# jaehyuck0103/OpenMAVIS

Hardware: AMD Instinct MI355X
Metric: multi-cam frames/sec (ORB extract+match) + LocalBA iters/sec, 5x720x540 (higher is better)
Workload: dtype u8

## Files before the change

include/omv.h:

```cpp
#ifndef OMV_H
#define OMV_H

#include <stddef.h>
#include <stdint.h>

#ifdef __cplusplus
extern "C" {
#endif

typedef int omv_status;
#define OMV_OK 0
#define OMV_ERR_ARG 1
#define OMV_ERR_HIP 2
#define OMV_ERR_CAPACITY 3
#define OMV_ERR_NO_DEVICE 4

typedef struct omv_orb_params {
    int nfeatures;
    float scale_factor;
    int nlevels;
    int ini_th_fast;
    int min_th_fast;
} omv_orb_params;

// ... 34 lines not shown
omv_status omv_orb_debug_level(omv_orb *orb, int img, int level, uint8_t *out, int *w, int *h);

typedef struct omv_frame_geom {
    int n_cams;
    float min_x, max_x;
    float min_y, max_y;
    int nlevels;
    float scale_factors[16];
    int cam_model[8];
} omv_frame_geom;

typedef struct omv_mp_view {
    const uint8_t *desc;
    const float *proj_x;
    const float *proj_y;
    const float *view_cos;
    const int32_t *level;
    const uint8_t *in_view;
    const float *track_depth;
    const uint8_t *is_bad;
    const uint8_t *has_obs;
} omv_mp_view;

typedef struct omv_matcher omv_matcher;

omv_status omv_matcher_create(int max_frames, int n_cams, int kp_cap, int max_mps, omv_matcher **out);
omv_status omv_matcher_destroy(omv_matcher *m);

omv_status omv_matcher_assign_grid(omv_matcher *m, int n_frames, const omv_frame_geom *geom, const omv_kp *kps,
                                   const int *n_kp, void *stream);
omv_status omv_matcher_grid_debug(omv_matcher *m, int frame, int cam, int32_t *cell_start, int32_t *idx);

omv_status omv_matcher_search_projection(omv_matcher *m, int n_frames, const omv_frame_geom *geom, const omv_kp *kps,
                                         const uint8_t *desc, const int *n_kp, const omv_mp_view *mps, int M, float th,
                                         int far_points, float th_far, float nnratio, const int32_t *l2r,
                                         const int32_t *r2l, const uint8_t *kp_occ_init, int32_t *kp_to_mp,
                                         int *n_matches, void *stream);

omv_status omv_matcher_stereo_lapping(omv_matcher *m, int n_frames, const uint8_t *desc, const int *n_kp,
                                      const int *mono, double ratio, int32_t *l2r, int32_t *r2l, void *stream);

omv_status omv_matcher_stereo_triangulate(omv_matcher *m, int n_frames, int n_cams, int kp_cap, const omv_kp *kps,
                                          const int *n_kp, const int *mono, const float *cams, const float *Rlr,
                                          const float *tlr, const float *level_sigma2, int nlevels, int32_t *l2r,
                                          int32_t *r2l, float *depth, float *p3d, void *stream);

omv_status omv_matcher_last_error(omv_matcher *m);

omv_status omv_matcher_enable_timing(omv_matcher *m, int on);
omv_status omv_matcher_stage_ms(omv_matcher *m, double *ms4, int reset);

omv_status omv_bf_knn2(int n_pairs, const uint8_t *query, int q_cap, const int *nq, const uint8_t *train, int t_cap,
                       const int *nt, int32_t *idx2, int32_t *dist2, void *stream);

typedef struct omv_se3f {
    float q[4];
    float t[3];
} omv_se3f;

typedef struct omv_last_frame {
    const float *pos;
    const uint8_t *desc;
    const uint8_t *valid;
    const uint8_t *has_obs;
    const omv_kp *kps;
    int S;
} omv_last_frame;

omv_status omv_matcher_search_last_frame(omv_matcher *m, int n_frames, const omv_frame_geom *geom, const omv_kp *kps,
                                         const uint8_t *desc, const int *n_kp, const float *cams, const omv_se3f *Tcw,
                                         const omv_se3f *Tlw, const omv_se3f *Trl, const omv_last_frame *last, float th,
                                         int bMono, float mb, int check_ori, const uint8_t *kp_occ_init,
                                         int32_t *kp_to_mp, int32_t *n_matches, void *stream);

enum { OMV_KF_FUSE = 0, OMV_KF_FUSE_SIM3 = 1, OMV_KF_SBP_SIM3 = 2, OMV_KF_SBP_FRAME = 3 };

typedef struct omv_kf_search_job {
    int kf;
    int cam;
    omv_se3f Tcw;
    float Ow[3];
    int mp_start, mp_count;
} omv_kf_search_job;

typedef struct omv_kf_mps {
    const float *pos;
    const float *normal;
    const float *min_dist;
    const float *max_dist;
    const uint8_t *desc;
} omv_kf_mps;

typedef struct omv_kf_search_params {
    int mode;
    float th;
    float max_dist;
    float bf;
    const float *uright;
    float inv_level_sigma2[16];
    float log_scale_factor;
    int n_levels;
    float cams[8][8];
    int check_ori;
    const float *mp_angle;
} omv_kf_search_params;

// ... 458 lines not shown
```

openmavis_amd/_lib.py:

```python
import ctypes
import os

_HERE = os.path.dirname(os.path.abspath(__file__))
LIB_PATH = os.path.join(_HERE, "libomv_hip.so")

OMV_OK = 0
OMV_ERR_ARG = 1
OMV_ERR_HIP = 2
OMV_ERR_CAPACITY = 3
OMV_ERR_NO_DEVICE = 4
CAM_KB8 = 0
CAM_PINHOLE = 1
_ERRS = {1: "bad argument", 2: "HIP runtime error", 3: "device capacity exceeded", 4: "no HIP device"}


class OmvError(RuntimeError):
    pass


def check(status, what="omv call"):
    if status != OMV_OK:
        raise OmvError(f"{what} failed: {_ERRS.get(status, status)} ({status})")


# ... 167 lines not shown

class FisheyeUndist(ctypes.Structure):
    _fields_ = [("K", ctypes.c_float * 4), ("D", ctypes.c_double * 4), ("newK", ctypes.c_float * 4)]


class LbaOpts(ctypes.Structure):
    _fields_ = [("opt_it", ctypes.c_int), ("lambda_init", ctypes.c_double), ("max_trials", ctypes.c_int),
                ("large", ctypes.c_int)]


class LbaResult(ctypes.Structure):
    _fields_ = [("err", ctypes.c_float), ("err_end", ctypes.c_float), ("status", ctypes.c_int),
                ("iterations", ctypes.c_int), ("trials", ctypes.c_int), ("lambda_", ctypes.c_double),
                ("mono_chi2", ctypes.c_void_p), ("mono_outlier", ctypes.c_void_p),
                ("stereo_chi2", ctypes.c_void_p), ("stereo_outlier", ctypes.c_void_p)]


try:
    import numpy as _np

    KP_DTYPE = _np.dtype([("x", "<f4"), ("y", "<f4"), ("size", "<f4"), ("angle", "<f4"),
                          ("response", "<f4"), ("octave", "<i4")])
except ImportError:
    KP_DTYPE = None

_VP, _I, _F, _SZ = ctypes.c_void_p, ctypes.c_int, ctypes.c_float, ctypes.c_size_t
ALLREDUCE_FN = ctypes.CFUNCTYPE(ctypes.c_int, ctypes.c_void_p, ctypes.c_void_p, ctypes.c_size_t, ctypes.c_void_p)
SIGNATURES = {
    "omv_orb_create": (_I, [ctypes.POINTER(OrbParams), _I, _I, _I, ctypes.POINTER(_VP)]),
    "omv_orb_destroy": (_I, [_VP]),
    "omv_selftest_node_sort": (_I, [_VP, _VP, _I, _VP, _VP]),
    "omv_orb_max_keypoints": (_I, [_VP]),
    "omv_orb_scale_tables": (_I, [_VP, _VP, _VP, _VP, _VP]),
    "omv_orb_extract_batch": (_I, [_VP, _I, _VP, _SZ, _SZ, _VP, _VP, _VP, _VP, _VP, _VP]),
    "omv_orb_extract_host": (_I, [_VP, _VP, _SZ, _I, _I, _VP, _VP, _VP, _VP]),
    "omv_orb_last_error": (_I, [_VP]),
    "omv_orb_enable_timing": (_I, [_VP, _I]),
    "omv_orb_set_harris": (_I, [_VP, _VP]),
    "omv_orb_stage_ms": (_I, [_VP, _VP, ctypes.POINTER(ctypes.c_longlong), _I]),
    "omv_orb_last_counts": (_I, [_VP, ctypes.POINTER(ctypes.c_longlong), ctypes.POINTER(ctypes.c_longlong)]),
    "omv_orb_debug_level": (_I, [_VP, _I, _I, _VP, ctypes.POINTER(_I), ctypes.POINTER(_I)]),
    "omv_matcher_create": (_I, [_I, _I, _I, _I, ctypes.POINTER(_VP)]),
    "omv_matcher_destroy": (_I, [_VP]),
    "omv_matcher_assign_grid": (_I, [_VP, _I, ctypes.POINTER(FrameGeom), _VP, _VP, _VP]),
    "omv_matcher_grid_debug": (_I, [_VP, _I, _I, _VP, _VP]),
    "omv_matcher_enable_timing": (_I, [_VP, _I]),
    "omv_matcher_last_error": (_I, [_VP]),
    "omv_matcher_stage_ms": (_I, [_VP, _VP, _I]),
    "omv_matcher_search_projection": (_I, [_VP, _I, ctypes.POINTER(FrameGeom), _VP, _VP, _VP,
                                           ctypes.POINTER(MpView), _I, _F, _I, _F, _F, _VP, _VP, _VP, _VP,
                                           _VP, _VP]),
    "omv_matcher_stereo_lapping": (_I, [_VP, _I, _VP, _VP, _VP, ctypes.c_double, _VP, _VP, _VP]),
    "omv_bf_knn2": (_I, [_I, _VP, _I, _VP, _VP, _I, _VP, _VP, _VP, _VP]),
    "omv_matcher_search_last_frame": (_I, [_VP, _I, ctypes.POINTER(FrameGeom), _VP, _VP, _VP, _VP, _VP, _VP,
                                           ctypes.POINTER(SE3f), ctypes.POINTER(LastFrame), _F, _I, _F, _I, _VP, _VP,
                                           _VP, _VP]),
    "omv_frustum": (_I, [_I, _VP, ctypes.POINTER(Rig), ctypes.POINTER(MpWorld), _I, _F, ctypes.POINTER(MpTrack), _VP,
                         _VP]),
    "omv_lba_create": (_I, [_I, _I, _I, _I, _I, ctypes.POINTER(_VP)]),
    "omv_lba_destroy": (_I, [_VP]),
    "omv_lba_set_problem": (_I, [_VP, ctypes.POINTER(LbaProblem)]),
    "omv_lba_optimize": (_I, [_VP, ctypes.POINTER(LbaOpts), ctypes.POINTER(LbaProblem), ctypes.POINTER(LbaResult)]),
    "omv_lba_evaluate": (_I, [_VP, _VP, _VP, _VP, _VP]),
    "omv_lba_evaluate_stereo": (_I, [_VP, _VP, _VP, _VP]),
    "omv_lba_stage_ms": (_I, [_VP, _VP, ctypes.POINTER(_I)]),
    "omv_lba_host_syncs": (_I, [_VP, ctypes.POINTER(_I), ctypes.POINTER(_I)]),
    "omv_lba_enable_timing": (_I, [_VP, _I]),
    "omv_lba_set_driver": (_I, [_VP, _I]),
    "omv_lba_reset": (_I, [_VP]),
    "omv_lba_set_comm": (_I, [_VP, _I, _I, _VP, _VP]),
    "omv_tri_debug": (_I, [_VP, _VP, _VP, _VP, _VP, _VP, _F, _F, _VP]),
    "omv_matcher_stereo_triangulate": (_I, [_VP, _I, _I, _I, _VP, _VP, _VP, _VP, _VP, _VP, _VP, _I, _VP, _VP, _VP,
                                            _VP, _VP]),
    "omv_matcher_search_for_triangulation": (_I, [_VP, _I, ctypes.POINTER(TriPair), _VP, _VP, _I, _I, _I, _VP, _VP]),
    "omv_matcher_search_by_bow": (_I, [_VP, _I, ctypes.POINTER(BowJob), _I, _F, _I, _VP, _VP]),
    "omv_matcher_bow_rescans": (_I, [ctypes.POINTER(ctypes.c_int64), _I]),
    "omv_matcher_search_for_initialization": (_I, [_VP, _I, _VP, ctypes.POINTER(FrameGeom), _VP, _VP, _VP, _VP, _I,
                                                   _F, _I, _VP, _VP, _VP]),
    "omv_pose_create": (_I, [_I, _I, ctypes.POINTER(_VP)]),
    "omv_pose_destroy": (_I, [_VP]),
    "omv_pose_inertial_last_kf": (_I, [_VP, ctypes.POINTER(PoseBatch), _I, _VP, _VP, _VP, _VP]),
    "omv_pose_inertial_last_frame": (_I, [_VP, ctypes.POINTER(PoseBatch), ctypes.POINTER(PosePrior), _I, _VP, _VP,
                                          _VP, _VP]),
    "omv_pose_constraint": (_I, [_I, _VP, _VP, _VP]),
    "omv_pose_optimization": (_I, [_VP, ctypes.POINTER(PoseBatch), _VP, _VP, _VP, _VP, _VP, _VP, _VP]),
    "omv_pose_set_mode": (_I, [_VP, _I, _I]),
    "omv_pose_edges_from_matches": (_I, [_VP, _I, _I, _VP, _VP, _VP, _VP, _VP, _VP, _I, _VP, _I] + [_VP] * 14),
    "omv_pose_last_error": (_I, [_VP, ctypes.POINTER(ctypes.c_int32), _VP]),
    "omv_matcher_search_kf": (_I, [_VP, _I, ctypes.POINTER(FrameGeom), _VP, _VP, _VP, _I, ctypes.POINTER(KfSearchJob),
                                   _I, _VP, ctypes.POINTER(KfMps), ctypes.POINTER(KfSearchParams), _VP, _VP, _VP, _VP,
                                   _VP]),
    "omv_search_in_neighbors_fuse": (_I, [_VP, ctypes.POINTER(FrameGeom), _VP, _VP, _VP, _I, ctypes.POINTER(FuseGraph),
                                          _I, _I, _VP, ctypes.POINTER(KfMps), ctypes.POINTER(KfSearchParams), _VP, _VP]),
    "omv_matcher_search_by_sim3": (_I, [_VP, _I, ctypes.POINTER(FrameGeom), _VP, _VP, _VP, _I, ctypes.POINTER(Sim3Job),
                                        _I, _VP, _VP, _I, _VP, _VP, ctypes.POINTER(KfMps), _F, _F, _I, _VP, _VP, _VP]),
    "omv_imu_preintegrate": (_I, [_I, _VP, _VP, _VP, _VP, _VP, _VP, _VP]),
    "omv_bow_transform": (_I, [ctypes.POINTER(Vocab), _I, _VP, _I, _VP, _I] + [_VP] * 10 + [_VP]),
    "omv_lba_shard": (_I, [_VP, ctypes.POINTER(ctypes.c_int32), ctypes.POINTER(ctypes.c_int32), _VP]),
    "omv_frame_uright": (_I, [_I, _I, _I, _I, _VP, _VP, _VP, _I, _I, ctypes.POINTER(FisheyeUndist), _F, _VP, _VP,
                              _VP]),
    "omv_frame_pack": (_I, [_I, _I, _I, _I, _VP, _VP, _VP, _VP, _VP, _VP, _VP, _VP, _VP]),
    "omv_mappoint_distinctive_descriptors": (_I, [_I, _VP, _VP, _VP, _VP, _VP, _VP]),
    "omv_create_new_map_points": (_I, [_I, _VP, _VP, _VP, _VP, _I, _I, _I, ctypes.c_float, ctypes.c_float, _I, _VP,
                                       _VP, _VP]),
    "omv_local_mapping_create_new_map_points": (_I, [_VP, _VP, _VP, _I, _VP, _VP, _VP, _I, _I, _I, _I, _I,
                                                     ctypes.c_float, ctypes.c_float, _VP, _VP, _VP]),
# ... 74 lines not shown
```

openmavis_amd/csrc/match.hip:

```cpp
#include <hip/hip_runtime.h>

#include <climits>
#include <cstdlib>
#include <cstring>
#include <type_traits>
#include <cmath>
#include <cstdio>
#include <vector>

#include "../../include/omv.h"
#include "omv_camera.h"
#include "omv_device.h"
#include "omv_host.h"

namespace {

constexpr int kGridCols = 64, kGridRows = 48, kCells = kGridCols * kGridRows;
constexpr int kTH_HIGH = 100;
constexpr int kTop = 16;
constexpr int kMaxCams = 8;
constexpr size_t kResolveLds = 150 * 1024;

struct FrameArgs {
    int n_cams, kp_cap, nlevels;
// ... 1070 lines not shown
    const int *q_off, *t_off;
    int pair_stride_off;
    int32_t *idx2, *dist2;
    int out_cap;
};

template <int G>
__global__ void __launch_bounds__(256) knn2_kernel(KnnArgs a, int n_pairs) {
    __shared__ __attribute__((aligned(16))) uint64_t tile[256][4];
    constexpr int QB = 256 / G;
    const int pair = blockIdx.y;
    const int qo = a.q_off ? a.q_off[pair * a.pair_stride_off] : 0;
    const int to = a.t_off ? a.t_off[pair * a.pair_stride_off] : 0;
    const int nq = a.nq[pair * a.pair_stride_off] - qo;
    const int nt = a.nt[pair * a.pair_stride_off] - to;
    const int g = threadIdx.x % G;
    const int qi = blockIdx.x * QB + threadIdx.x / G;
    if (blockIdx.x * QB >= max(nq, 0)) return;
    uint64_t dq[4] = {0, 0, 0, 0};
    if (qi < nq) omv::load_desc(a.q + pair * a.q_stride + (size_t)(qo + qi) * 32, dq);
    uint64_t k0 = ~0ull >> 1, k1 = ~0ull >> 1;
    int d0 = INT_MAX, d1 = INT_MAX, i0 = -1, i1 = -1;
    for (int b = 0; b < nt; b += 256) {
        __syncthreads();
        const int j = b + threadIdx.x;
        if (j < nt) omv::load_desc(a.t + pair * a.t_stride + (size_t)(to + j) * 32, tile[threadIdx.x]);
        __syncthreads();
        const int e = min(256, nt - b);
        for (int k = g; k < e; k += G) {
            const int d = omv::hamming256(dq, tile[k]);
            if (d < d1) {
                if (d0 > d) d1 = d0, i1 = i0, d0 = d, i0 = b + k;
                else d1 = d, i1 = b + k;
            }
        }
    }
    k0 = ((uint64_t)(uint32_t)d0 << 32) | (uint32_t)i0;
    k1 = ((uint64_t)(uint32_t)d1 << 32) | (uint32_t)i1;
#pragma unroll
    for (int m = 1; m < G; m <<= 1) {
        const uint64_t o0 = __shfl_xor(k0, m, 64), o1 = __shfl_xor(k1, m, 64);
        const uint64_t r0 = k0 < o0 ? k0 : o0;
        const uint64_t r1 = k0 < o0 ? (k1 < o0 ? k1 : o0) : (k0 < o1 ? k0 : o1);
        k0 = r0, k1 = r1;
    }
    if (qi < nq && g == 0) {
        int32_t *oi = a.idx2 + ((size_t)pair * a.out_cap + qi) * 2;
        int32_t *od = a.dist2 + ((size_t)pair * a.out_cap + qi) * 2;
        oi[0] = (int32_t)(uint32_t)k0, oi[1] = (int32_t)(uint32_t)k1;
        od[0] = (int32_t)(k0 >> 32), od[1] = (int32_t)(k1 >> 32);
    }
}

static void launch_knn2(const KnnArgs &a, int n_pairs, int q_cap, hipStream_t st) {
    if ((long long)n_pairs * q_cap <= 4096)
        knn2_kernel<32><<<dim3((q_cap + 7) / 8, n_pairs), 256, 0, st>>>(a, n_pairs);
    else
        knn2_kernel<8><<<dim3((q_cap + 31) / 32, n_pairs), 256, 0, st>>>(a, n_pairs);
}

__global__ void stereo_pairs_kernel(const int32_t *idx2, const int32_t *dist2, int out_cap, const int *n_kp,
                                    const int *mono, int n_cams, int kp_cap, double ratio, int32_t *l2r,
                                    int32_t *r2l, int n_frames) {
    const int frame = blockIdx.y;
    const int q = blockIdx.x * blockDim.x + threadIdx.x;
    if (q >= kp_cap) return;
    const int m0 = mono[frame * n_cams], m1 = mono[frame * n_cams + 1];
    const int nq = n_kp[frame * n_cams] - m0, qi = q - m0;
    int32_t v = -1;
    if (qi >= 0 && qi < nq) {
        const int32_t *oi = idx2 + ((size_t)frame * out_cap + qi) * 2;
        const int32_t *od = dist2 + ((size_t)frame * out_cap + qi) * 2;
        if (oi[1] >= 0 && (double)od[0] < (double)od[1] * ratio) {
            v = m1 + oi[0];
            atomicMax(&r2l[(size_t)frame * kp_cap + m1 + oi[0]], q);
        }
    }
    l2r[(size_t)frame * kp_cap + q] = v;
}

__device__ __forceinline__ void mat3f(const float *a, const float *b, float *r) {
    for (int i = 0; i < 3; ++i)
        for (int j = 0; j < 3; ++j) r[3 * i + j] = a[3 * i] * b[j] + a[3 * i + 1] * b[3 + j] + a[3 * i + 2] * b[6 + j];
}
__device__ __forceinline__ void matvec3f(const float *a, const float *x, float *r) {
    for (int i = 0; i < 3; ++i) r[i] = a[3 * i] * x[0] + a[3 * i + 1] * x[1] + a[3 * i + 2] * x[2];
}

__global__ void __launch_bounds__(256) frustum_kernel(const omv_frame_pose *poses, omv_rig rig, omv_mp_world mp, int M,
                                                      float cos_limit, omv_mp_track out, int32_t *n_in_view) {
    __shared__ float Rc[kMaxCams][9], tc[kMaxCams][3], twc[kMaxCams][3];
    const int frame = blockIdx.y, C = rig.n_cams;
    const omv_frame_pose &pose = poses[frame];
    if (threadIdx.x < C) {
        const int c = threadIdx.x;
        if (c == 0) {
            for (int q = 0; q < 9; ++q) Rc[0][q] = pose.Rcw[q];
            for (int q = 0; q < 3; ++q) tc[0][q] = pose.tcw[q], twc[0][q] = pose.Ow[q];
        } else {
            float R[9], t[3];
            mat3f(rig.R_cl[c], pose.Rcw, R);
            for (int q = 0; q < 9; ++q) Rc[c][q] = R[q];
            matvec3f(rig.R_cl[c], pose.tcw, t);
            for (int q = 0; q < 3; ++q) tc[c][q] = t[q] + rig.t_cl[c][q];
            matvec3f(pose.Rwc, rig.t_lc[c], t);
            for (int q = 0; q < 3; ++q) twc[c][q] = t[q] + pose.Ow[q];
        }
    }
// ... 935 lines not shown
    f.kps = kps, f.desc = desc, f.n_kp = n_kp;
    f.cell_start = h->d_cell_start, f.cell_idx = h->d_cell_idx;
}

constexpr size_t kResolveStaticLds = 4 * ((size_t)kMaxDomains * (2 * kListCap + kMaxRevived + 2) + 1);
static size_t resolve_lds_bytes(int C, int cap, int M, int *lds_k2m = nullptr) {
    const size_t S = (size_t)C * cap;
    const size_t b = sizeof(uint32_t) * 2 * ((S + 31) / 32) + sizeof(int) * S + 2 * sizeof(int32_t) * cap + ((size_t)M + 3) / 4 * 4;
    const size_t with_k2m = b + sizeof(int32_t) * S;
    const bool fits = with_k2m + kResolveStaticLds <= kResolveLds;
    if (lds_k2m) *lds_k2m = fits;
    return fits ? with_k2m : b;
}
static size_t lf_resolve_lds_bytes(int C, int cap) {
    const size_t S = (size_t)C * cap;
    return sizeof(uint32_t) * ((S + 31) / 32) + sizeof(int) * S;
}

extern "C" {

omv_status omv_frustum(int n_frames, const omv_frame_pose *poses, const omv_rig *rig, const omv_mp_world *mp, int M,
                       float viewing_cos_limit, const omv_mp_track *out, int32_t *n_in_view, void *stream) {
    if (n_frames <= 0 || !poses || !rig || !mp || !out || M < 0 || rig->n_cams <= 0 || rig->n_cams > kMaxCams ||
        rig->n_levels <= 0 || !cam_models_ok(rig->model, rig->n_cams))
        return OMV_ERR_ARG;
    if (M == 0) return OMV_OK;
    hipStream_t st = (hipStream_t)stream;
    frustum_kernel<<<dim3((M + 255) / 256, n_frames), 256, 0, st>>>(poses, *rig, *mp, M, viewing_cos_limit, *out,
                                                                    n_in_view);
    HIP_OK(hipGetLastError());
    return OMV_OK;
}

omv_status omv_matcher_create(int max_frames, int n_cams, int kp_cap, int max_mps, omv_matcher **out) {
    if (!out || max_frames <= 0 || n_cams <= 0 || n_cams > kMaxCams || kp_cap <= 0 || kp_cap > 65535 || max_mps < 0)
        return OMV_ERR_ARG;
    if (resolve_lds_bytes(n_cams, kp_cap, max_mps) > kResolveLds - kResolveStaticLds || lf_resolve_lds_bytes(n_cams, kp_cap) > kResolveLds)
        return OMV_ERR_ARG;
    int ndev = 0;
    if (hipGetDeviceCount(&ndev) != hipSuccess || ndev == 0) return OMV_ERR_NO_DEVICE;
    const int resolve_dyn = (int)(kResolveLds - kResolveStaticLds);
    HIP_OK(hipFuncSetAttribute((const void *)resolve_kernel<true>, hipFuncAttributeMaxDynamicSharedMemorySize, resolve_dyn));
    HIP_OK(hipFuncSetAttribute((const void *)resolve_kernel<false>, hipFuncAttributeMaxDynamicSharedMemorySize, resolve_dyn));
    HIP_OK(hipFuncSetAttribute((const void *)lf_resolve_kernel, hipFuncAttributeMaxDynamicSharedMemorySize, (int)kResolveLds));
    HIP_OK(hipFuncSetAttribute((const void *)cand_stage_kernel, hipFuncAttributeMaxDynamicSharedMemorySize, (int)kStageLdsMax));
    auto h = std::make_unique<omv_matcher>();
    h->max_frames = max_frames, h->n_cams = n_cams, h->kp_cap = kp_cap, h->max_mps = max_mps;
    if (const char *e = getenv("OMV_BOW_TOP")) h->knobs.bow_top = atoi(e);
    if (const char *e = getenv("OMV_TRI_SLICES")) h->knobs.tri_slices = atoi(e);
    if (const char *e = getenv("OMV_TRI_ECAP")) h->knobs.tri_ecap = atoi(e);
    if (const char *e = getenv("OMV_TRI_WALK")) h->knobs.tri_walk_seq = strcmp(e, "seq") == 0 ? 1 : 0;
    if (const char *e = getenv("OMV_CAND")) h->knobs.cand_mode = strcmp(e, "global") == 0 ? 1 : strcmp(e, "lds") == 0 ? 2 : 0;
    if (const char *e = getenv("OMV_CAND_PW")) h->knobs.cand_pw = atoi(e);
    const size_t fc = (size_t)max_frames * n_cams;
    const size_t knn = (size_t)2 * max_frames * kp_cap;
    omv::DeviceArena &mem = h->mem;
    if (!mem.alloc(&h->d_cell_start, fc * (kCells + 1)) || !mem.alloc(&h->d_cell_idx, fc * kp_cap) ||
        !mem.alloc(&h->d_recs, fc * max_mps) || !mem.alloc(&h->d_counts, fc * max_mps) ||
        !mem.alloc(&h->d_flags, (size_t)max_frames * max_mps) || !mem.alloc(&h->d_knn_i, knn) ||
        !mem.alloc(&h->d_knn_d, knn) || !mem.alloc(&h->d_err, 1))
        return OMV_ERR_HIP;
    HIP_OK(hipMemset(h->d_err, 0, sizeof(int)));
    *out = h.release();
    return OMV_OK;
}

omv_status omv_matcher_enable_timing(omv_matcher *h, int on) {
    if (!h) return OMV_ERR_ARG;
    h->timing = on != 0;
    return OMV_OK;
}

omv_status omv_matcher_stage_ms(omv_matcher *h, double *ms4, int reset) {
    if (!h || !ms4) return OMV_ERR_ARG;
    HIP_OK(hipStreamSynchronize(h->last));
    for (auto &p : h->ev) {
        float ms = 0.f;
        (void)hipEventElapsedTime(&ms, p.second.first, p.second.second);
        h->stage_ms[p.first] += ms;
        (void)hipEventDestroy(p.second.first);
        (void)hipEventDestroy(p.second.second);
    }
    h->ev.clear();
    for (int k = 0; k < 4; ++k) ms4[k] = h->stage_ms[k];
    if (reset)
        for (int k = 0; k < 4; ++k) h->stage_ms[k] = 0;
    return OMV_OK;
}

omv_status omv_matcher_last_error(omv_matcher *h) {
    if (!h) return OMV_ERR_ARG;
    HIP_OK(hipStreamSynchronize(h->last));
    int e = 0;
    HIP_OK(hipMemcpy(&e, h->d_err, sizeof(int), hipMemcpyDeviceToHost));
    HIP_OK(hipMemset(h->d_err, 0, sizeof(int)));
    return e;
}

omv_status omv_matcher_destroy(omv_matcher *h) {
    if (!h) return OMV_ERR_ARG;
    delete h;
    return OMV_OK;
}

omv_status omv_matcher_assign_grid(omv_matcher *h, int n_frames, const omv_frame_geom *g, const omv_kp *kps,
                                   const int *n_kp, void *stream) {
// ... 183 lines not shown
                                      const uint8_t *desc, const int *n_kp, int n_jobs, const omv_sim3_job *jobs,
                                      int n1, const int32_t *kp1, const int32_t *mp1, int n2, const int32_t *kp2,
                                      const int32_t *mp2, const omv_kf_mps *mps, float th, float log_scale_factor,
                                      int n_levels, int32_t *match12, int32_t *n_found, void *stream) {
    if (!h || !g || !kps || !desc || !n_kp || !mps || n_kf <= 0 || n_kf > h->max_frames || g->n_cams != h->n_cams ||
        n_jobs < 0 || n1 < 0 || n2 < 0 || (n_jobs > 0 && (!jobs || !n_found)) || (n1 > 0 && (!kp1 || !mp1 || !match12)) ||
        (n2 > 0 && (!kp2 || !mp2)) || ((n1 + n2) > 0 && (!mps->pos || !mps->desc || !mps->min_dist || !mps->max_dist)) ||
        n_levels <= 0 || n_levels > 16)
        return OMV_ERR_ARG;
    int next1 = 0, next2 = 0;
    for (int j = 0; j < n_jobs; ++j) {
        const omv_sim3_job &J = jobs[j];
        if (J.kf1 < 0 || J.kf1 >= n_kf || J.kf2 < 0 || J.kf2 >= n_kf || J.start1 != next1 || J.count1 < 0 ||
            J.start2 != next2 || J.count2 < 0)
            return OMV_ERR_ARG;
        next1 += J.count1, next2 += J.count2;
    }
    if (next1 != n1 || next2 != n2) return OMV_ERR_ARG;
    if (!cam_models_ok(g->cam_model, h->n_cams)) return OMV_ERR_ARG;
    if (n_jobs == 0) return OMV_OK;
    hipStream_t st = (hipStream_t)stream;
    h->last = st;
    const int N = h->n_cams * h->kp_cap;
    const size_t job_b = ((sizeof(omv_sim3_job) * n_jobs + 255) / 256) * 256;
    const size_t vn1_b = ((sizeof(int32_t) * std::max(1, n1) + 255) / 256) * 256;
    const size_t vn2_b = sizeof(int32_t) * (size_t)n_jobs * N;
    omv::DeviceArena ws;
    uint8_t *buf = nullptr;
    if (!ws.alloc_async(&buf, job_b + vn1_b + vn2_b, st)) return OMV_ERR_HIP;
    Sim3Args a{};
    fill_frame(h, g, kps, desc, n_kp, a.f);
    a.jobs = reinterpret_cast<const omv_sim3_job *>(buf);
    a.n_jobs = n_jobs, a.n1 = n1, a.n2 = n2, a.N = N;
    a.kp1 = kp1, a.mp1 = mp1, a.kp2 = kp2, a.mp2 = mp2, a.mps = *mps;
    a.th = th, a.log_scale = log_scale_factor, a.n_levels = n_levels;
    a.vn1 = reinterpret_cast<int32_t *>(buf + job_b);
    a.vn2 = reinterpret_cast<int32_t *>(buf + job_b + vn1_b);
    a.match12 = match12, a.n_found = n_found;
    HIP_OK(hipMemcpyAsync(buf, jobs, sizeof(omv_sim3_job) * n_jobs, hipMemcpyHostToDevice, st));
    HIP_OK(hipMemsetAsync(a.vn2, 0xff, vn2_b, st));
    HIP_OK(hipMemsetAsync(n_found, 0, sizeof(int32_t) * n_jobs, st));
    if (n1 + n2 > 0) sbs3_cand_kernel<<<(n1 + n2 + 255) / 256, 256, 0, st>>>(a);
    if (n1 > 0) sbs3_agree_kernel<<<(n1 + 255) / 256, 256, 0, st>>>(a);
    HIP_OK(hipGetLastError());
    HIP_OK(ws.free(&buf));
    return OMV_OK;
}

omv_status omv_bf_knn2(int n_pairs, const uint8_t *query, int q_cap, const int *nq, const uint8_t *train, int t_cap,
                       const int *nt, int32_t *idx2, int32_t *dist2, void *stream) {
    if (n_pairs <= 0 || !query || !train || !nq || !nt || !idx2 || !dist2 || q_cap <= 0 || t_cap <= 0)
        return OMV_ERR_ARG;
    KnnArgs a{query, train, (long long)q_cap * 32, (long long)t_cap * 32, nq, nt, nullptr, nullptr, 1, idx2, dist2, q_cap};
    launch_knn2(a, n_pairs, q_cap, (hipStream_t)stream);
    HIP_OK(hipGetLastError());
    return OMV_OK;
}

omv_status omv_matcher_stereo_lapping(omv_matcher *h, int n_frames, const uint8_t *desc, const int *n_kp,
                                      const int *mono, double ratio, int32_t *l2r, int32_t *r2l, void *stream) {
    if (!h || h->n_cams < 2 || !desc || !n_kp || !mono || !l2r || !r2l || n_frames <= 0 || n_frames > h->max_frames)
        return OMV_ERR_ARG;
    hipStream_t st = (hipStream_t)stream;
    h->last = st;
    const int cap = h->kp_cap, C = h->n_cams;
    hipEvent_t e0 = h->timing ? mk_event(st) : nullptr;
    HIP_OK(hipMemsetAsync(r2l, 0xff, sizeof(int32_t) * n_frames * cap, st));
    KnnArgs a{desc, desc + (size_t)cap * 32, (long long)C * cap * 32, (long long)C * cap * 32, n_kp, n_kp + 1,
              mono, mono + 1, C, h->d_knn_i, h->d_knn_d, cap};
    launch_knn2(a, n_frames, cap, st);
    dim3 g2((cap + 255) / 256, n_frames);
    stereo_pairs_kernel<<<g2, 256, 0, st>>>(h->d_knn_i, h->d_knn_d, cap, n_kp, mono, C, cap, ratio, l2r, r2l, n_frames);
    if (h->timing) h->ev.push_back({1, {e0, mk_event(st)}});
    HIP_OK(hipGetLastError());
    return OMV_OK;
}


omv_status omv_matcher_search_for_initialization(omv_matcher *h, int n_pairs, const int32_t *pairs,
                                                 const omv_frame_geom *g, const omv_kp *kps, const uint8_t *desc,
                                                 const int *n_kp, float *prev_matched, int window, float nnratio,
                                                 int check_ori, int32_t *matches12, int32_t *n_matches, void *stream) {
    if (!h || n_pairs < 0 || (n_pairs > 0 && (!pairs || !g || !kps || !desc || !n_kp || !prev_matched || !matches12 ||
                                              !n_matches)) ||
        g->n_cams != h->n_cams || window < 0)
        return OMV_ERR_ARG;
    if (n_pairs == 0) return OMV_OK;
    for (int i = 0; i < 2 * n_pairs; ++i)
        if (pairs[i] < 0 || pairs[i] >= h->max_frames) return OMV_ERR_ARG;
    hipStream_t st = (hipStream_t)stream;
    h->last = st;
    FrameArgs f;
    if (!cam_models_ok(g->cam_model, h->n_cams)) return OMV_ERR_ARG;
    fill_frame(h, g, kps, desc, n_kp, f);
    const size_t lds = init_lds_bytes(h->kp_cap);
    if (lds > 160 * 1024) return OMV_ERR_CAPACITY;
    HIP_OK(hipFuncSetAttribute((const void *)init_kernel, hipFuncAttributeMaxDynamicSharedMemorySize, (int)lds));
    omv::DeviceArena ws;
    int32_t *d_pairs = nullptr;
    if (!ws.alloc_async(&d_pairs, (size_t)2 * n_pairs, st)) return OMV_ERR_HIP;
    HIP_OK(hipMemcpyAsync(d_pairs, pairs, sizeof(int32_t) * 2 * n_pairs, hipMemcpyHostToDevice, st));
    uint4 *d_spec = nullptr;
    if (!ws.alloc_async(&d_spec, 4 * (size_t)n_pairs * h->kp_cap, st)) return OMV_ERR_HIP;
    InitArgs ia{f, d_pairs, prev_matched, window, nnratio, check_ori, matches12, n_matches, d_spec};
    init_spec_kernel<<<dim3((h->kp_cap + 3) / 4, n_pairs), 256, 0, st>>>(ia);
    init_kernel<<<n_pairs, 64, lds, st>>>(ia);
    HIP_OK(hipGetLastError());
    HIP_OK(ws.free(&d_spec));
    HIP_OK(ws.free(&d_pairs));
    return OMV_OK;
}

}
```

openmavis_amd/csrc/omv_device.h:

```cpp
#pragma once
#include <hip/hip_runtime.h>
#include <stdint.h>

#include "omv_math.h"

namespace omv {


__device__ __forceinline__ int reflect101(int p, int n) {
    p = p < 0 ? -p : p;
    return p >= n ? 2 * n - 2 - p : p;
}

__device__ __forceinline__ int hamming256(const uint64_t *a, const uint64_t *b) {
    return __popcll(a[0] ^ b[0]) + __popcll(a[1] ^ b[1]) + __popcll(a[2] ^ b[2]) + __popcll(a[3] ^ b[3]);
}
__device__ __forceinline__ void load_desc(const uint8_t *p, uint64_t d[4]) {
    const uint64_t *q = reinterpret_cast<const uint64_t *>(p);
    d[0] = q[0], d[1] = q[1], d[2] = q[2], d[3] = q[3];
}

__device__ __forceinline__ void wave_lds_sync() {
    __builtin_amdgcn_fence(__ATOMIC_RELEASE, "wavefront");
    __builtin_amdgcn_wave_barrier();
    __builtin_amdgcn_fence(__ATOMIC_ACQUIRE, "wavefront");
}

__device__ __forceinline__ double rcp_nr(double x) {
    double r = __builtin_amdgcn_rcp(x);
    double e = __builtin_fma(-x, r, 1.0);
    r = __builtin_fma(r, e, r);
    e = __builtin_fma(-x, r, 1.0);
    return __builtin_fma(r, e, r);
}


__device__ __forceinline__ int xcd_block(int n_logical) {
    const int chunk = (n_logical + 7) >> 3;
    const int b = (int)(blockIdx.x & 7) * chunk + (int)(blockIdx.x >> 3);
    return b < n_logical ? b : -1;
}
__host__ inline int xcd_grid(int n_logical) { return (n_logical + 7) & ~7; }

}
extern "C" __device__ __attribute__((const)) uint32_t omv_llvm_mul_u24(uint32_t, uint32_t) __asm("llvm.amdgcn.mul.u24.i32");
extern "C" __device__ __attribute__((const)) uint32_t omv_llvm_mulhi_u24(uint32_t, uint32_t) __asm("llvm.amdgcn.mulhi.u24");
namespace omv {
__device__ __forceinline__ int mul_u24(int a, int b) { return (int)omv_llvm_mul_u24((uint32_t)a, (uint32_t)b); }
__device__ __forceinline__ uint32_t mulhi_u24(uint32_t a, uint32_t b) { return omv_llvm_mulhi_u24(a, b); }

struct MatcherKnobs {
    int bow_top = -1, tri_slices = -1, tri_ecap = -1, tri_walk_seq = 0;
    int cand_mode = 0;
    int cand_pw = -1;
};
MatcherKnobs matcher_knobs(const struct ::omv_matcher *m);
size_t matcher_kf_entry_cap(const struct ::omv_matcher *m);

}
```

openmavis_amd/matcher.py:

```python
import ctypes

import numpy as np

from . import _lib

FRAME_GRID_COLS = 64
FRAME_GRID_ROWS = 48
TH_HIGH = 100
TH_LOW = 50
HISTO_LENGTH = 30


def frame_geom(n_cams, width, height, scale_factors, cam_model=None):
    g = _lib.FrameGeom()
    g.n_cams = n_cams
    g.min_x, g.max_x, g.min_y, g.max_y = 0.0, float(width), 0.0, float(height)
    g.nlevels = len(scale_factors)
    for i, s in enumerate(scale_factors):
        g.scale_factors[i] = float(s)
    for i, m in enumerate(cam_model if cam_model is not None else ()):
        g.cam_model[i] = {"kb8": _lib.CAM_KB8, "pinhole": _lib.CAM_PINHOLE}.get(m, m) if isinstance(m, str) else int(m)
    return g


# ... 351 lines not shown
    for i in range(c.shape[0]):
        for q in range(8):
            p.cams[i][q] = float(c[i, q])
    p.mp_angle = _lib.ptr(mp_angle) if mp_angle is not None else None
    p._keep = (uright, mp_angle)
    return p


def make_rig(cams, R_cl, t_cl, width, height, scale_factor=1.2, nlevels=8, model="kb8"):
    r = _lib.Rig()
    C = len(cams)
    r.n_cams = C
    models = [model] * C if isinstance(model, str) else list(model)
    for c in range(C):
        r.model[c] = {"kb8": _lib.CAM_KB8, "pinhole": _lib.CAM_PINHOLE}[models[c]]
        for q in range(len(cams[c])):
            r.cam[c][q] = float(cams[c][q])
        Rc = np.asarray(R_cl[c], np.float32).reshape(3, 3)
        tc = np.asarray(t_cl[c], np.float32).reshape(3)
        tlc = (-(Rc.astype(np.float64).T @ tc.astype(np.float64))).astype(np.float32)
        for q in range(9):
            r.R_cl[c][q] = float(Rc.reshape(-1)[q])
        for q in range(3):
            r.t_cl[c][q] = float(tc[q])
            r.t_lc[c][q] = float(tlc[q]) if c else 0.0
    r.min_x, r.max_x, r.min_y, r.max_y = 0.0, float(width), 0.0, float(height)
    r.log_scale_factor = float(np.float32(np.log(np.float64(np.float32(scale_factor)))))
    r.n_levels = nlevels
    return r


def isInFrustum(poses, rig, world, track, viewingCosLimit=0.5, n_in_view=None, stream=None):
    lib = _lib.load()
    F, M = world["pos"].shape[0], world["pos"].shape[1]
    w = _lib.MpWorld(_lib.ptr(world["pos"]), _lib.ptr(world["normal"]), _lib.ptr(world["min_dist"]),
                     _lib.ptr(world["max_dist"]))
    t = _lib.MpTrack(_lib.ptr(track.proj_x), _lib.ptr(track.proj_y), _lib.ptr(track.view_cos), _lib.ptr(track.level),
                     _lib.ptr(track.in_view), _lib.ptr(track.track_depth))
    s = ctypes.c_void_p(stream.cuda_stream) if stream is not None else None
    _lib.check(lib.omv_frustum(F, _lib.ptr(poses), ctypes.byref(rig), ctypes.byref(w), M, ctypes.c_float(viewingCosLimit),
                               ctypes.byref(t), _lib.ptr(n_in_view), s), "omv_frustum")


def bf_knn2(query, nq, train, nt, stream=None):
    import torch
    lib = _lib.load()
    P, Q = query.shape[0], query.shape[1]
    idx2 = torch.empty((P, Q, 2), dtype=torch.int32, device=query.device)
    dist2 = torch.empty((P, Q, 2), dtype=torch.int32, device=query.device)
    s = ctypes.c_void_p(stream.cuda_stream) if stream is not None else None
    _lib.check(lib.omv_bf_knn2(P, _lib.ptr(query), Q, _lib.ptr(nq), _lib.ptr(train), train.shape[1], _lib.ptr(nt),
                               _lib.ptr(idx2), _lib.ptr(dist2), s), "omv_bf_knn2")
    return idx2, dist2
```

Measured before the change: 48230.

## Compute brute-force Hamming kNN2 with int8 MFMA on ±1-expanded descriptors

Result: faster. 48970, median of 6 (+1.5%).

```diff
diff --git a/include/omv.h b/include/omv.h
--- a/include/omv.h
+++ b/include/omv.h
@@ -110,6 +110,7 @@
 
 omv_status omv_bf_knn2(int n_pairs, const uint8_t *query, int q_cap, const int *nq, const uint8_t *train, int t_cap,
                        const int *nt, int32_t *idx2, int32_t *dist2, void *stream);
+int omv_bf_knn2_path(int n_pairs, int q_cap, int t_cap);
 
 typedef struct omv_se3f {
     float q[4];
diff --git a/openmavis_amd/_lib.py b/openmavis_amd/_lib.py
--- a/openmavis_amd/_lib.py
+++ b/openmavis_amd/_lib.py
@@ -243,6 +243,7 @@
                                            _VP, _VP]),
     "omv_matcher_stereo_lapping": (_I, [_VP, _I, _VP, _VP, _VP, ctypes.c_double, _VP, _VP, _VP]),
     "omv_bf_knn2": (_I, [_I, _VP, _I, _VP, _VP, _I, _VP, _VP, _VP, _VP]),
+    "omv_bf_knn2_path": (_I, [_I, _I, _I]),
     "omv_matcher_search_last_frame": (_I, [_VP, _I, ctypes.POINTER(FrameGeom), _VP, _VP, _VP, _VP, _VP, _VP,
                                            ctypes.POINTER(SE3f), ctypes.POINTER(LastFrame), _F, _I, _F, _I, _VP, _VP,
                                            _VP, _VP]),
diff --git a/openmavis_amd/csrc/match.hip b/openmavis_amd/csrc/match.hip
--- a/openmavis_amd/csrc/match.hip
+++ b/openmavis_amd/csrc/match.hip
@@ -1146,8 +1146,133 @@
     }
 }
 
-static void launch_knn2(const KnnArgs &a, int n_pairs, int q_cap, hipStream_t st) {
-    if ((long long)n_pairs * q_cap <= 4096)
+constexpr int kKnnTile = 64;
+constexpr int kKnnRowB = 256 + 16;
+constexpr uint32_t kKnnNone = ~0u;
+typedef int knn_i32x4 __attribute__((ext_vector_type(4)));
+
+__device__ __forceinline__ uint32_t knn_spread4(uint32_t w, int d) {
+    return omv_llvm_mul_u24((w >> (4 * d)) & 15u, 0x204081u) & 0x01010101u;
+}
+template <bool pm>
+__device__ __forceinline__ knn_i32x4 knn_expand16(uint32_t bits) {
+    knn_i32x4 r;
+#pragma unroll
+    for (int d = 0; d < 4; ++d) {
+        const uint32_t y = knn_spread4(bits, d);
+        r[d] = (int)(pm ? ((0x80808080u - y) ^ 0x80808080u) | 0x01010101u : y);
+    }
+    return r;
+}
+__device__ __forceinline__ uint32_t knn_med3(uint32_t a, uint32_t b, uint32_t c) {
+    uint32_t r;
+    asm("v_med3_u32 %0, %1, %2, %3" : "=v"(r) : "v"(a), "v"(b), "v"(c));
+    return r;
+}
+
+__global__ void __launch_bounds__(256, 2) knn2_mfma_kernel(KnnArgs a, int n_pairs) {
+    __shared__ __attribute__((aligned(16))) uint8_t tile[kKnnTile * kKnnRowB];
+    const int pair = blockIdx.y;
+    const int qo = a.q_off ? a.q_off[pair * a.pair_stride_off] : 0;
+    const int to = a.t_off ? a.t_off[pair * a.pair_stride_off] : 0;
+    const int nq = a.nq[pair * a.pair_stride_off] - qo;
+    const int nt = a.nt[pair * a.pair_stride_off] - to;
+    if ((int)blockIdx.x * 256 >= max(nq, 0)) return;
+    const int lane = threadIdx.x & 63, c = lane & 15, h = lane >> 4;
+    const int qb = blockIdx.x * 256 + (threadIdx.x >> 6) * 64;
+    const bool live = qb < nq;
+    knn_i32x4 bq[4][4];
+    int pq[4];
+    uint32_t k0[4], k1[4];
+#pragma unroll
+    for (int ct = 0; ct < 4; ++ct) {
+        const int qi = qb + 16 * ct + c;
+        uint64_t dq[4] = {0, 0, 0, 0};
+        if (qi < nq) omv::load_desc(a.q + pair * a.q_stride + (size_t)(qo + qi) * 32, dq);
+        pq[ct] = __popcll(dq[0]) + __popcll(dq[1]) + __popcll(dq[2]) + __popcll(dq[3]);
+#pragma unroll
+        for (int s = 0; s < 4; ++s) bq[ct][s] = knn_expand16<true>((uint32_t)(dq[s] >> (16 * h)) & 0xffffu);
+        k0[ct] = k1[ct] = kKnnNone;
+    }
+    const uint8_t *tbase = a.t + pair * a.t_stride + (size_t)to * 32;
+    const int sr = threadIdx.x >> 2, sw = threadIdx.x & 3;
+    auto score = [&](int b, auto full) {
+#pragma unroll
+        for (int rt = 0; rt < kKnnTile / 16; ++rt) {
+            knn_i32x4 ta[4];
+#pragma unroll
+            for (int s = 0; s < 4; ++s)
+                ta[s] = *reinterpret_cast<const knn_i32x4 *>(tile + (16 * rt + c) * kKnnRowB + s * 64 + h * 16);
+            const int row = b + 16 * rt + 4 * h;
+#pragma unroll
+            for (int ct = 0; ct < 4; ++ct) {
+                knn_i32x4 acc = {pq[ct], pq[ct], pq[ct], pq[ct]};
+#pragma unroll
+                for (int s = 0; s < 4; ++s) acc = __builtin_amdgcn_mfma_i32_16x16x64_i8(ta[s], bq[ct][s], acc, 0, 0, 0);
+#pragma unroll
+                for (int i = 0; i < 4; ++i) {
+                    uint32_t k = ((uint32_t)acc[i] << 16) | (uint32_t)(row + i);
+                    if (!decltype(full)::value) k = row + i < nt ? k : kKnnNone;
+                    k1[ct] = knn_med3(k, k0[ct], k1[ct]);
+                    k0[ct] = min(k, k0[ct]);
+                }
+            }
+        }
+    };
+    for (int b = 0; b < nt; b += kKnnTile) {
+        __syncthreads();
+        {
+            const int j = b + sr;
+            const uint64_t v = j < nt ? *reinterpret_cast<const uint64_t *>(tbase + (size_t)j * 32 + sw * 8) : 0ull;
+            knn_i32x4 *dst = reinterpret_cast<knn_i32x4 *>(tile + sr * kKnnRowB + sw * 64);
+#pragma unroll
+            for (int i = 0; i < 4; ++i) dst[i] = knn_expand16<false>((uint32_t)(v >> (16 * i)) & 0xffffu);
+        }
+        __syncthreads();
+        if (!live) continue;
+        if (b + kKnnTile <= nt) score(b, std::true_type{});
+        else score(b, std::false_type{});
+    }
+    if (!live) return;
+#pragma unroll
+    for (int ct = 0; ct < 4; ++ct) {
+        uint32_t m0 = k0[ct], m1 = k1[ct];
+#pragma unroll
+        for (int m = 16; m < 64; m <<= 1) {
+            const uint32_t o0 = __shfl_xor(m0, m, 64), o1 = __shfl_xor(m1, m, 64);
+            const uint32_t r0 = min(m0, o0);
+            const uint32_t r1 = m0 < o0 ? min(m1, o0) : min(m0, o1);
+            m0 = r0, m1 = r1;
+        }
+        const int qi = qb + 16 * ct + c;
+        if (qi < nq && h == 0) {
+            int32_t *oi = a.idx2 + ((size_t)pair * a.out_cap + qi) * 2;
+            int32_t *od = a.dist2 + ((size_t)pair * a.out_cap + qi) * 2;
+            oi[0] = m0 == kKnnNone ? -1 : (int32_t)(m0 & 0xffffu), oi[1] = m1 == kKnnNone ? -1 : (int32_t)(m1 & 0xffffu);
+            od[0] = m0 == kKnnNone ? INT_MAX : (int32_t)(m0 >> 16), od[1] = m1 == kKnnNone ? INT_MAX : (int32_t)(m1 >> 16);
+        }
+    }
+}
+
+constexpr int kKnnIdxLimit = 1 << 16;
+static int knn_mode_env() {
+    const char *e = getenv("OMV_KNN");
+    return !e ? 0 : strcmp(e, "mfma") == 0 ? 1 : strcmp(e, "lanes") == 0 ? 2 : 0;
+}
+static int knn_idx_limit_env() {
+    const char *e = getenv("OMV_KNN_IDX_LIMIT");
+    const int v = e ? atoi(e) : 0;
+    return v > 0 && v < kKnnIdxLimit ? v : kKnnIdxLimit;
+}
+static bool knn_use_mfma(int mode, int idx_limit, int n_pairs, int q_cap, int t_cap) {
+    if (t_cap >= idx_limit) return false;
+    return mode == 1 || (mode == 0 && (long long)n_pairs * q_cap > 4096);
+}
+
+static void launch_knn2(const KnnArgs &a, int n_pairs, int q_cap, int t_cap, int mode, int idx_limit, hipStream_t st) {
+    if (knn_use_mfma(mode, idx_limit, n_pairs, q_cap, t_cap))
+        knn2_mfma_kernel<<<dim3((q_cap + 255) / 256, n_pairs), 256, 0, st>>>(a, n_pairs);
+    else if ((long long)n_pairs * q_cap <= 4096)
         knn2_kernel<32><<<dim3((q_cap + 7) / 8, n_pairs), 256, 0, st>>>(a, n_pairs);
     else
         knn2_kernel<8><<<dim3((q_cap + 31) / 32, n_pairs), 256, 0, st>>>(a, n_pairs);
@@ -2189,6 +2314,7 @@
     if (const char *e = getenv("OMV_TRI_WALK")) h->knobs.tri_walk_seq = strcmp(e, "seq") == 0 ? 1 : 0;
     if (const char *e = getenv("OMV_CAND")) h->knobs.cand_mode = strcmp(e, "global") == 0 ? 1 : strcmp(e, "lds") == 0 ? 2 : 0;
     if (const char *e = getenv("OMV_CAND_PW")) h->knobs.cand_pw = atoi(e);
+    h->knobs.knn_mode = knn_mode_env(), h->knobs.knn_idx_limit = knn_idx_limit_env();
     const size_t fc = (size_t)max_frames * n_cams;
     const size_t knn = (size_t)2 * max_frames * kp_cap;
     omv::DeviceArena &mem = h->mem;
@@ -2478,9 +2604,13 @@
     if (n_pairs <= 0 || !query || !train || !nq || !nt || !idx2 || !dist2 || q_cap <= 0 || t_cap <= 0)
         return OMV_ERR_ARG;
     KnnArgs a{query, train, (long long)q_cap * 32, (long long)t_cap * 32, nq, nt, nullptr, nullptr, 1, idx2, dist2, q_cap};
-    launch_knn2(a, n_pairs, q_cap, (hipStream_t)stream);
+    launch_knn2(a, n_pairs, q_cap, t_cap, knn_mode_env(), knn_idx_limit_env(), (hipStream_t)stream);
     HIP_OK(hipGetLastError());
     return OMV_OK;
+}
+
+int omv_bf_knn2_path(int n_pairs, int q_cap, int t_cap) {
+    return knn_use_mfma(knn_mode_env(), knn_idx_limit_env(), n_pairs, q_cap, t_cap) ? 1 : 0;
 }
 
 omv_status omv_matcher_stereo_lapping(omv_matcher *h, int n_frames, const uint8_t *desc, const int *n_kp,
@@ -2494,7 +2624,7 @@
     HIP_OK(hipMemsetAsync(r2l, 0xff, sizeof(int32_t) * n_frames * cap, st));
     KnnArgs a{desc, desc + (size_t)cap * 32, (long long)C * cap * 32, (long long)C * cap * 32, n_kp, n_kp + 1,
               mono, mono + 1, C, h->d_knn_i, h->d_knn_d, cap};
-    launch_knn2(a, n_frames, cap, st);
+    launch_knn2(a, n_frames, cap, cap, h->knobs.knn_mode, h->knobs.knn_idx_limit, st);
     dim3 g2((cap + 255) / 256, n_frames);
     stereo_pairs_kernel<<<g2, 256, 0, st>>>(h->d_knn_i, h->d_knn_d, cap, n_kp, mono, C, cap, ratio, l2r, r2l, n_frames);
     if (h->timing) h->ev.push_back({1, {e0, mk_event(st)}});
diff --git a/openmavis_amd/csrc/omv_device.h b/openmavis_amd/csrc/omv_device.h
--- a/openmavis_amd/csrc/omv_device.h
+++ b/openmavis_amd/csrc/omv_device.h
@@ -53,6 +53,8 @@
     int bow_top = -1, tri_slices = -1, tri_ecap = -1, tri_walk_seq = 0;
     int cand_mode = 0;
     int cand_pw = -1;
+    int knn_mode = 0;
+    int knn_idx_limit = 1 << 16;
 };
 MatcherKnobs matcher_knobs(const struct ::omv_matcher *m);
 size_t matcher_kf_entry_cap(const struct ::omv_matcher *m);
diff --git a/openmavis_amd/matcher.py b/openmavis_amd/matcher.py
--- a/openmavis_amd/matcher.py
+++ b/openmavis_amd/matcher.py
@@ -427,3 +427,7 @@
     _lib.check(lib.omv_bf_knn2(P, _lib.ptr(query), Q, _lib.ptr(nq), _lib.ptr(train), train.shape[1], _lib.ptr(nt),
                                _lib.ptr(idx2), _lib.ptr(dist2), s), "omv_bf_knn2")
     return idx2, dist2
+
+
+def bf_knn2_path(n_pairs, q_cap, t_cap):
+    return "mfma" if _lib.load().omv_bf_knn2_path(n_pairs, q_cap, t_cap) else "lanes"
```
